# huangnengCSU/NanoSNP

Hardware: AMD Instinct MI355X
Metric: candidate SNP sites/sec (pileup encode + model fwd), 30x windows (higher is better)
Workload: dtype f32; 1 GPU; BASELINE configs[1]: pileup encode + PileupModel fwd, 1M synthetic 30x windows (G2) resident in HBM, batch=4096; batch=4096, windows_resident_per_gpu=1048576, streams=32, precision=fp32, parallelism=site-sharded x1, rooted gather of calls, world_size_observed=1, gather=torch

## Files before the change

nanosnp_amd/csrc/nsnp_api.hip:

```cpp
#include "nsnp_common.hpp"

#include <new>

extern "C" int nsnp_version(void) { return 100; }

extern "C" const char* nsnp_strerror(int code)
{
    switch (code) {
    case NSNP_OK: return "ok";
    case NSNP_EINVAL: return "invalid argument";
    case NSNP_ENOMEM: return "out of memory";
    case NSNP_EHIP: return "HIP runtime error";
    case NSNP_ENOWEIGHTS: return "weights not loaded";
    case NSNP_EARCH: return "device is not gfx950";
    case NSNP_ESHAPE: return "unsupported model dimensions";
    case NSNP_ENOTSUP: return "optional component unavailable (RCCL not found)";
    case NSNP_ECOMM: return "RCCL call failed";
    default: return "unknown error";
    }
}

static hipError_t g_create_err = hipSuccess;

extern "C" int nsnp_last_hip_error(const nsnp_ctx* ctx, const char** text)
{
    const hipError_t e = ctx ? ctx->last_err : g_create_err;
    if (text) *text = hipGetErrorString(e);
    return (int)e;
}

extern "C" int nsnp_ctx_create(int device, nsnp_ctx** out)
{
    if (!out) return NSNP_EINVAL;
    *out = nullptr;
    nsnp_ctx* ctx = new (std::nothrow) nsnp_ctx();
    if (!ctx) return NSNP_ENOMEM;
    memset((void*)ctx, 0, sizeof(*ctx));
    ctx->device = device;
    ctx->last_err = hipSuccess;
    ctx->chunk_sites = 32768;
    ctx->hap_chunk = 16384;
    ctx->precision = 0;
    ctx->hap_precision = 0;
    ctx->cat_precision = 0;
    ctx->cat_conv_lds = 1;
    ctx->cat_conv_pix2 = 1;
    ctx->hap_b3x = 1;
    ctx->tok_fused = 0;
    ctx->proj1_tiles = 4;
    ctx->fused_l1 = 1;
    ctx->l0_rs = 1;
    ctx->l1_rs = 1;
    ctx->l1_stagger = 0;
    ctx->head_rs = 1;
    ctx->rs_prio = 0;
    hipDeviceProp_t prop;
    hipError_t e = hipSetDevice(device);
    if (e == hipSuccess) e = hipGetDeviceProperties(&prop, device);
    if (e != hipSuccess) { g_create_err = e; delete ctx; return NSNP_EHIP; }
    if (strncmp(prop.gcnArchName, "gfx950", 6) != 0) { delete ctx; return NSNP_EARCH; }
    ctx->n_cu = prop.multiProcessorCount;
    *out = ctx;
    return NSNP_OK;
}

void nsnp_hap_free(nsnp_ctx* ctx);
int  nsnp_hap_reserve(nsnp_ctx* ctx);
void nsnp_cat_free(nsnp_ctx* ctx);
void nsnp_tok_free(nsnp_ctx* ctx);

constexpr size_t TIMER_MAX_PAIRS = 8192;

ScopedKernelTimer::ScopedKernelTimer(nsnp_ctx* c, int kernel, hipStream_t stream)
    : ctx(c), k(kernel), s(stream), stop_ev(nullptr), on(false)
{
    KernelTimer* t = c->timer;
    if (!t || !t->enabled || t->used[k] >= TIMER_MAX_PAIRS) return;
    if (t->used[k] == t->start[k].size()) {
        hipEvent_t a, b;
        if (hipEventCreate(&a) != hipSuccess) return;
        if (hipEventCreate(&b) != hipSuccess) { (void)hipEventDestroy(a); return; }
        t->start[k].push_back(a); t->stop[k].push_back(b);
    }
    const size_t i = t->used[k]++;
    (void)hipEventRecord(t->start[k][i], s);
    stop_ev = t->stop[k][i];
    on = true;
}
void ScopedKernelTimer::stop() { if (on) { (void)hipEventRecord(stop_ev, s); on = false; } }
ScopedKernelTimer::~ScopedKernelTimer() { stop(); }

extern "C" int nsnp_ctx_set_option(nsnp_ctx* ctx, const char* name, int64_t value)
{
    if (!ctx || !name) return NSNP_EINVAL;
    if (strcmp(name, "cat_precision") == 0) {
        if (value != 0 && value != 1 && value != 2) return NSNP_EINVAL;
        ctx->cat_precision = (int)value;
        return NSNP_OK;
    }
    if (strcmp(name, "tok_fused") == 0) {
        if (value != 0 && value != 1) return NSNP_EINVAL;
        ctx->tok_fused = (int)value;
        return NSNP_OK;
    }
    if (strcmp(name, "hap_b3x") == 0) {
        if (value != 0 && value != 1) return NSNP_EINVAL;
        ctx->hap_b3x = (int)value;
        return NSNP_OK;
    }
    if (strcmp(name, "cat_conv_pix2") == 0) {
        if (value != 0 && value != 1) return NSNP_EINVAL;
        ctx->cat_conv_pix2 = (int)value;
        return NSNP_OK;
    }
    if (strcmp(name, "cat_conv_lds") == 0) {
        if (value != 0 && value != 1) return NSNP_EINVAL;
        ctx->cat_conv_lds = (int)value;
        return NSNP_OK;
    }
    if (strcmp(name, "hap_precision") == 0) {
        if (value != 0 && value != 1 && value != 2) return NSNP_EINVAL;
        ctx->hap_precision = (int)value;
        return nsnp_hap_reserve(ctx);
    }
    if (strcmp(name, "hap_pass_sites") == 0) {
        if (value < 128 || value > 131072 || value % 128) return NSNP_EINVAL;
        const int64_t old = ctx->hap_chunk;
        ctx->hap_chunk = value;
        const int rc = nsnp_hap_reserve(ctx);
        if (rc) { ctx->hap_chunk = old; (void)nsnp_hap_reserve(ctx); }
        return rc;
    }
    if (strcmp(name, "pileup_precision") == 0) {
        if (value != 0 && value != 1 && value != 2) return NSNP_EINVAL;
        ctx->precision = (int)value;
        if (value == 2 && ctx->ws_h0 && ctx->ws_h0_floats < 192) return nsnp_ctx_reserve(ctx, ctx->chunk_sites);
        return NSNP_OK;
    }
    if (strcmp(name, "fused_l1") == 0) {
        if (value != 0 && value != 1) return NSNP_EINVAL;
        ctx->fused_l1 = (int)value;
        return NSNP_OK;
    }
    if (strcmp(name, "l0_register_stationary") == 0) {
        if (value != 0 && value != 1) return NSNP_EINVAL;
        ctx->l0_rs = (int)value;
        return NSNP_OK;
    }
    if (strcmp(name, "l1_register_stationary") == 0) {
        if (value != 0 && value != 1 && value != 2) return NSNP_EINVAL;
        ctx->l1_rs = (int)value;
        return NSNP_OK;
    }
    if (strcmp(name, "l0_input_weights_in_lds") == 0) {
        if (value != 0 && value != 1) return NSNP_EINVAL;
        ctx->l0_wx_lds = (int)value;
        return NSNP_OK;
    }
    if (strcmp(name, "static_priority") == 0) {
        if (value < 0 || value > 3) return NSNP_EINVAL;
        ctx->rs_prio = (int)value;
        return NSNP_OK;
    }
    if (strcmp(name, "head_split") == 0) {
        if (value != 0 && value != 1) return NSNP_EINVAL;
        ctx->head_rs = (int)value;
        return NSNP_OK;
    }
    if (strcmp(name, "l1_stagger") == 0) {
        if (value != 0 && value != 1) return NSNP_EINVAL;
        ctx->l1_stagger = (int)value;
        return NSNP_OK;
    }
    if (strcmp(name, "l1_site_groups") == 0) {
        if (value != 0 && value != 1 && value != 2 && value != 4) return NSNP_EINVAL;
        ctx->l1_rs_groups = (int)value;
        return NSNP_OK;
    }
    if (strcmp(name, "l0_site_groups") == 0) {
        if (value != 0 && value != 1 && value != 2 && value != 4) return NSNP_EINVAL;
        ctx->l0_rs_groups = (int)value;
        return NSNP_OK;
    }
    if (strcmp(name, "fused_waves") == 0) {
        if (value != 0 && value != 4 && value != 8 && value != 12) return NSNP_EINVAL;
        ctx->fused_waves = (int)value;
        return NSNP_OK;
    }
    if (strcmp(name, "proj1_tiles") == 0) {
        if (value < 1 || value > 64) return NSNP_EINVAL;
        ctx->proj1_tiles = (int)value;
        return NSNP_OK;
    }
    if (strcmp(name, "recurrence_waves") == 0) {
        if (value != 0 && value != 1 && value != 2 && value != 4 && value != 8) return NSNP_EINVAL;
        ctx->force_wpb = (int)value;
        return NSNP_OK;
    }
// ... 163 lines not shown
```

nanosnp_amd/csrc/nsnp_common.hpp:

```cpp
#pragma once

#include <hip/hip_runtime.h>
#include <stdint.h>
#include <stdlib.h>
#include <string.h>
#include <vector>

#include "nanosnp.h"

typedef float f32x4 __attribute__((ext_vector_type(4)));
typedef int   i32x4 __attribute__((ext_vector_type(4)));

#define NSNP_CDIV(a, b) (((a) + (b) - 1) / (b))

constexpr int PW = NSNP_PILEUP_WINDOW;
constexpr int PC = NSNP_PILEUP_CHANNELS;
constexpr int PH = 64;
constexpr int PG = 4 * PH;
constexpr int PCENTER = 16;
constexpr int PSTEPS1 = PCENTER + 1;


struct PileupWeightsDev {
    float* l0_whh[2];
    float* l0_wih[2];
    float* l0_wlast[2];
    float* l1_wih[2];
    float* l1_bias[2];
    float* l1_bias_raw[2];
    float* l1_whh[2];
    float* proj_w;
    float* proj_b;
    float* dense_w;
    float* dense_b;
    float* head_w;
    float* head_b;
    float* arena;
    size_t arena_bytes;
    bool   loaded;
};

struct PileupWeightsF16 {
    void* l0_whh[2]; void* l0_wih_hi[2]; void* l0_wih_lo[2]; void* l1_wih[2]; void* l1_whh[2];
    void* l1f_hi[2]; void* l1f_lo[2]; float* l1f_bias;
    void* l0_wih_rs[2];
    void* l1_wih_rs[2]; void* l1_whh_rs[2];
    void* l0_whh_rs[2];
    void* proj_w; void* dense_w; void* head_w;
    void* arena; size_t arena_bytes; bool loaded;
};

struct PileupWeightsB3 {
    void* l0_whh[2]; void* l0_wih[2]; void* l1_wih[2]; void* l1_whh[2];
    void* proj_w; void* dense_w; void* head_w;
    float* proj_b; float* dense_b; float* head_b;
    void* arena; size_t arena_bytes; bool loaded;
};

struct HapWeightsDev;
struct CatWeightsDev;

enum { NSNP_K_L0 = 0, NSNP_K_PROJ1, NSNP_K_L1, NSNP_K_HEAD, NSNP_K_ENCODE, NSNP_K_HAPFEAT, NSNP_K_HAPLSTM, NSNP_K_CATCONV, NSNP_K_CAT,
       NSNP_K_COUNT };
struct KernelTimer {
    std::vector<hipEvent_t> start[NSNP_K_COUNT], stop[NSNP_K_COUNT];
    size_t used[NSNP_K_COUNT];
    bool enabled;
};

struct PostOut { uint8_t* gt_arg; uint8_t* zy_arg; float* gt_max; float* zy_max; };

struct nsnp_ctx {
    int device;
    int n_cu;
    hipError_t last_err;
    bool attr_set;
    bool attr_set_f16;
    bool attr_set_b3;
    int hap_b3x;
// ... 68 lines not shown
```

nanosnp_amd/csrc/pileup_forward.hip:

```cpp
#include "nsnp_common.hpp"
#include "nsnp_lstm_cell.hpp"
#include "nsnp_devclock.hpp"

namespace {

constexpr float LOG2E = 1.4426950408889634f;

__device__ __forceinline__ f32x4 mfma4(float a, float b, f32x4 c)
{
    return __builtin_amdgcn_mfma_f32_16x16x4f32(a, b, c, 0, 0, 0);
}
__device__ __forceinline__ float sigmoid_f(float x)
{
    return __builtin_amdgcn_rcpf(1.0f + __builtin_amdgcn_exp2f(-LOG2E * x));
}
__device__ __forceinline__ float tanh_f(float x)
{
    return __builtin_fmaf(-2.0f, __builtin_amdgcn_rcpf(1.0f + __builtin_amdgcn_exp2f((2.0f * LOG2E) * x)), 1.0f);
}

__device__ __forceinline__ float lstm_cell(float zi, float zf, float zg, float zo, float& c)
{
    float cn;
    const float h = nsnp_cell::lstm_cell(zi, zf, zg, zo, c, cn);
    c = cn;
    return h;
}

template <int NT, int NJ4, int J4B, int J4N, int TB = 0, typename WP>
__device__ __forceinline__ void wave_gemm(WP w, int lane, const float* b, f32x4* acc)
{
#pragma unroll
    for (int j = 0; j < J4N; ++j) {
#pragma unroll
        for (int ig = 0; ig < NT; ig += 4) {
            f32x4 a[4];
#pragma unroll
            for (int u = 0; u < 4; ++u) a[u] = w[((TB + ig + u) * NJ4 + (J4B + j)) * 64 + lane];
#pragma unroll
            for (int e = 0; e < 4; ++e)
#pragma unroll
                for (int u = 0; u < 4; ++u) acc[ig + u] = mfma4(a[u][e], b[4 * j + e], acc[ig + u]);
            __builtin_amdgcn_sched_barrier(0);
        }
    }
}

__device__ __forceinline__ void wave_gemm2x16(const f32x4* w, int lane, const float* b, f32x4* acc)
{
#pragma unroll
    for (int j = 0; j < 16; ++j) {
        const f32x4 a0 = w[(0 * 16 + j) * 64 + lane], a1 = w[(1 * 16 + j) * 64 + lane];
#pragma unroll
        for (int e = 0; e < 4; ++e) {
            acc[0] = mfma4(a0[e], b[4 * j + e], acc[0]);
// ... 363 lines not shown
            const float* xr = &xx[cur][(16 * sg + n) * RS_XSROW];
            const f32x4 xb = *reinterpret_cast<const f32x4*>(xr + 4 * q);
            const float xl = xr[16 + q];
            f32x4 acc[4];
#pragma unroll
            for (int u = 0; u < 4; ++u) acc[u] = f32x4{0.f, 0.f, 0.f, 0.f};
            if (WXL) {
#pragma unroll
                for (int u = 0; u < 4; ++u) {
                    Wih[u] = *reinterpret_cast<const f32x4*>(&wxl[((wave * 4 + u) * 64 + lane) * 4]);
                    Wl[u] = wxl[4 * 4 * 64 * 4 + (wave * 4 + u) * 64 + lane];
                }
            }
#pragma unroll
            for (int e = 0; e < 4; ++e)
#pragma unroll
                for (int u = 0; u < 4; ++u) acc[u] = mfma4(Wih[u][e], xb[e], acc[u]);
#pragma unroll
            for (int u = 0; u < 4; ++u) acc[u] = mfma4(Wl[u], xl, acc[u]);
            if (s > 0) {
#define RS_KBLOCK(J, HB)                                                                               \
                _Pragma("unroll") for (int e = 0; e < 4; ++e)                                          \
                    _Pragma("unroll") for (int u = 0; u < 4; ++u) acc[u] = mfma4(Whh[u][J][e], HB[e], acc[u]);
                __builtin_amdgcn_sched_barrier(0);
                RS_KBLOCK(0, hb0)
                __builtin_amdgcn_sched_barrier(0);
                hb0 = *reinterpret_cast<const f32x4*>(hr + 32);
                RS_KBLOCK(1, hb1)
                __builtin_amdgcn_sched_barrier(0);
                hb1 = *reinterpret_cast<const f32x4*>(hr + 48);
                RS_KBLOCK(2, hb0)
                __builtin_amdgcn_sched_barrier(0);
                RS_KBLOCK(3, hb1)
#undef RS_KBLOCK
            }
            f32x4 hn;
#pragma unroll
            for (int u = 0; u < 4; ++u) {
                hn[u] = lstm_cell(acc[u][0], acc[u][1], acc[u][2], acc[u][3], c[sg][u]);
            }
            *reinterpret_cast<f32x4*>(&hx[cur][16 * sg + n][16 * wave + 4 * q]) = hn;
        }
        }
        if (s + 1 < PW) {
            stage_x(cur ^ 1);
            if (s + 2 < PW) load_x(dir ? t - 2 : t + 2);
        }
        lds_barrier();
    }
    flush_h((PW - 1) & 1, dir ? 0 : PW - 1);
    NSNP_DEVCLK_STOP(0)
}

constexpr int rs32_l1_lds_bytes(int nsg) { return (2 * 16 * nsg * RS_H0ROW + 2 * 16 * nsg * RS_XROW) * 4; }

template <int NSG, bool STAGGER>
__global__ __launch_bounds__(512, 2) void k_pileup_l1_rs32(
    const float* __restrict__ H0, int64_t N,
    const float* __restrict__ wih0, const float* __restrict__ wih1,
    const float* __restrict__ whh0, const float* __restrict__ whh1,
    const float* __restrict__ bias0, const float* __restrict__ bias1,
    float* __restrict__ H1c)
{
    extern __shared__ f32x4 lds[];
    constexpr int NS = 16 * NSG;
    float* const h0s = reinterpret_cast<float*>(lds);
    float* const h1x = h0s + 2 * NS * RS_H0ROW;
    const int dir = blockIdx.y;
    const int tid = threadIdx.x, lane = tid & 63, wave = tid >> 6;
    const int n = lane & 15, q = lane >> 4;
    const int64_t base_site = (int64_t)blockIdx.x * NS;

    f32x4 Wih[2][8], Whh[2][4], bias[2];
    {
        const f32x4* __restrict__ gih = reinterpret_cast<const f32x4*>(dir ? wih1 : wih0);
        const f32x4* __restrict__ ghh = reinterpret_cast<const f32x4*>(dir ? whh1 : whh0);
        const f32x4* __restrict__ gb = reinterpret_cast<const f32x4*>(dir ? bias1 : bias0);
#pragma unroll
        for (int u = 0; u < 2; ++u) {
#pragma unroll
            for (int j = 0; j < 8; ++j) Wih[u][j] = gih[((2 * wave + u) * 8 + j) * 64 + lane];
#pragma unroll
            for (int j = 0; j < 4; ++j) Whh[u][j] = ghh[((2 * wave + u) * 4 + j) * 64 + lane];
            bias[u] = gb[(2 * wave + u) * 64 + lane];
        }
    }

    const int cid = tid & 31;
    const int slot = (cid & 16) + 4 * (cid & 3) + ((cid >> 2) & 3);
    f32x4 sreg[NSG];
    auto load_h0 = [&](int t) {
#pragma unroll
        for (int k = 0; k < NSG; ++k) {
            const int64_t site = base_site + (tid >> 5) + 16 * k;
            const int64_t sc = site < N ? site : N - 1;
            sreg[k] = *reinterpret_cast<const f32x4*>(H0 + (sc * PW + t) * 128 + 4 * cid);
        }
    };
    auto store_h0 = [&](int buf) {
#pragma unroll
        for (int k = 0; k < NSG; ++k)
            *reinterpret_cast<f32x4*>(h0s + ((size_t)buf * NS + (tid >> 5) + 16 * k) * RS_H0ROW + 4 * slot) = sreg[k];
    };
    auto tpos = [&](int u) { return dir ? PW - 1 - u : u; };
    load_h0(tpos(0)); store_h0(0);
    load_h0(tpos(1)); store_h0(1);
// ... 446 lines not shown
        int d = 0;
        for (int k = 0; k < 8; ++k) { const int v = c[idx[k]]; if (v < 0) d -= v; }
        depth[n] = d;
    }
}

}

namespace {

inline int gate_row(int row)
{
    const int i = row >> 4, r = row & 15, qp = r >> 2, g = r & 3;
    return g * PH + 4 * i + qp;
}
struct MatRef { const float* w; int ld; const float* b0; const float* b1; };

float f_whh(const void* u, int row, int k) { const MatRef* m = (const MatRef*)u; return m->w[gate_row(row) * m->ld + k]; }
float f_wih0(const void* u, int row, int k) { const MatRef* m = (const MatRef*)u; return m->w[gate_row(row) * m->ld + k]; }
inline int h_store_col(int k) { const int j = k >> 2, q = k & 3; return (j >> 4) * 64 + 4 * (j & 15) + q; }
float f_wih1(const void* u, int row, int k) { const MatRef* m = (const MatRef*)u; return m->w[gate_row(row) * m->ld + h_store_col(k)]; }
float f_proj(const void* u, int row, int k) { const MatRef* m = (const MatRef*)u; return m->w[row * m->ld + h_store_col(k)]; }
inline int acc_col(int k) { const int j = k >> 2, q = k & 3; return 16 * (j >> 2) + 4 * q + (j & 3); }
float f_dense(const void* u, int row, int k) { const MatRef* m = (const MatRef*)u; return m->w[row * m->ld + acc_col(k)]; }
struct HeadRef { const float* gt; const float* zy; };
float f_head(const void* u, int row, int k)
{
    const HeadRef* m = (const HeadRef*)u;
    if (row < 21) return m->gt[row * 256 + acc_col(k)];
    if (row < 24) return m->zy[(row - 21) * 256 + acc_col(k)];
    return 0.f;
}

}

void nsnp_pack_image(float* img, int n_tiles, int n_j4, nsnp_wfun f, const void* user)
{
    for (int tile = 0; tile < n_tiles; ++tile)
        for (int j4 = 0; j4 < n_j4; ++j4)
            for (int lane = 0; lane < 64; ++lane)
                for (int e = 0; e < 4; ++e) {
                    const int row = 16 * tile + (lane & 15);
                    const int k = 4 * (4 * j4 + e) + (lane >> 4);
                    img[(((size_t)tile * n_j4 + j4) * 64 + lane) * 4 + e] = f(user, row, k);
                }
}

int nsnp_pileup_pack_weights(nsnp_ctx* ctx, const float* const* w)
{
    PileupWeightsDev& pw = ctx->pw;
    const size_t n_whh = 16 * 4 * 256, n_wih0 = 16 * 1 * 256, n_wlast = 16 * 64, n_wih1 = 16 * 8 * 256,
                 n_b1 = 16 * 256, n_proj = 8 * 8 * 256, n_pb = 8 * 256, n_dense = 16 * 8 * 256, n_db = 16 * 256,
                 n_head = 2 * 16 * 256, n_hb = 2 * 256;
    const size_t total = 2 * (n_whh + n_wih0 + n_wlast + n_wih1 + 2 * n_b1 + n_whh) + n_proj + n_pb + n_dense + n_db + n_head + n_hb;
    std::vector<float> host(total);
    size_t off = 0;
    auto take = [&](size_t n) { float* p = host.data() + off; off += n; return p; };
    float* h_l0_whh[2]; float* h_l0_wih[2]; float* h_l0_wlast[2]; float* h_l1_wih[2]; float* h_l1_b[2]; float* h_l1_braw[2]; float* h_l1_whh[2];
    for (int d = 0; d < 2; ++d) {
        h_l0_whh[d] = take(n_whh); h_l0_wih[d] = take(n_wih0); h_l0_wlast[d] = take(n_wlast);
        h_l1_wih[d] = take(n_wih1); h_l1_b[d] = take(n_b1); h_l1_braw[d] = take(n_b1); h_l1_whh[d] = take(n_whh);
    }
    float* h_proj = take(n_proj); float* h_pb = take(n_pb); float* h_dense = take(n_dense); float* h_db = take(n_db);
    float* h_head = take(n_head); float* h_hb = take(n_hb);

    std::vector<float> scaled[16];
    const float* ws[16];
    for (int t = 0; t < 16; ++t) {
        const int layer = t / 8, kind = t % 4;
        const size_t cols = kind == 0 ? (layer ? 2 * PH : PC) : (kind == 1 ? PH : 1);
        scaled[t].resize((size_t)4 * PH * cols);
        for (int r = 0; r < 4 * PH; ++r) {
            const float f = (r / PH == 2) ? -2.0f * LOG2E : -LOG2E;
            for (size_t k = 0; k < cols; ++k) scaled[t][r * cols + k] = f * w[t][r * cols + k];
        }
        ws[t] = scaled[t].data();
    }
    for (int d = 0; d < 2; ++d) {
        const float* const* l0 = ws + d * 4;
        const float* const* l1 = ws + 8 + d * 4;
        MatRef m;
        m = MatRef{l0[1], PH, nullptr, nullptr};  nsnp_pack_image(h_l0_whh[d], 16, 4, f_whh, &m);
        m = MatRef{l0[0], PC, nullptr, nullptr};  nsnp_pack_image(h_l0_wih[d], 16, 1, f_wih0, &m);
        for (int tile = 0; tile < 16; ++tile)
            for (int lane = 0; lane < 64; ++lane) {
                const int tr = gate_row(16 * tile + (lane & 15)), kq = lane >> 4;
                float v = 0.f;
                if (kq < 2) v = l0[0][tr * PC + 16 + kq];
                else if (kq == 2) v = l0[2][tr] + l0[3][tr];
                h_l0_wlast[d][tile * 64 + lane] = v;
            }
        m = MatRef{l1[0], 2 * PH, nullptr, nullptr};  nsnp_pack_image(h_l1_wih[d], 16, 8, f_wih1, &m);
        for (int tile = 0; tile < 16; ++tile)
            for (int lane = 0; lane < 64; ++lane)
                for (int g = 0; g < 4; ++g) {
                    const int tr = gate_row(16 * tile + 4 * (lane >> 4) + g);
                    h_l1_b[d][(tile * 64 + lane) * 4 + g] = l1[2][tr] + l1[3][tr];
                    h_l1_braw[d][(tile * 64 + lane) * 4 + g] = w[8 + d * 4 + 2][tr] + w[8 + d * 4 + 3][tr];
                }
        m = MatRef{l1[1], PH, nullptr, nullptr};  nsnp_pack_image(h_l1_whh[d], 16, 4, f_whh, &m);
    }
    {
        MatRef m{w[16], 128, nullptr, nullptr};  nsnp_pack_image(h_proj, 8, 8, f_proj, &m);
        for (int tile = 0; tile < 8; ++tile) for (int lane = 0; lane < 64; ++lane) for (int g = 0; g < 4; ++g)
            h_pb[(tile * 64 + lane) * 4 + g] = w[17][16 * tile + 4 * (lane >> 4) + g];
        MatRef md{w[18], 128, nullptr, nullptr}; nsnp_pack_image(h_dense, 16, 8, f_dense, &md);
        for (int tile = 0; tile < 16; ++tile) for (int lane = 0; lane < 64; ++lane) for (int g = 0; g < 4; ++g)
            h_db[(tile * 64 + lane) * 4 + g] = w[19][16 * tile + 4 * (lane >> 4) + g];
        HeadRef hr{w[20], w[22]};  nsnp_pack_image(h_head, 2, 16, f_head, &hr);
        for (int tile = 0; tile < 2; ++tile) for (int lane = 0; lane < 64; ++lane) for (int g = 0; g < 4; ++g) {
            const int row = 16 * tile + 4 * (lane >> 4) + g;
            h_hb[(tile * 64 + lane) * 4 + g] = row < 21 ? w[21][row] : (row < 24 ? w[23][row - 21] : 0.f);
        }
    }
    if (pw.arena && pw.arena_bytes != total * sizeof(float)) { (void)hipFree(pw.arena); pw.arena = nullptr; }
    if (!pw.arena) {
        NSNP_HIP(ctx, hipMalloc((void**)&pw.arena, total * sizeof(float)));
        pw.arena_bytes = total * sizeof(float);
    }
    NSNP_HIP(ctx, hipMemcpy(pw.arena, host.data(), total * sizeof(float), hipMemcpyHostToDevice));
    auto dev = [&](const float* hp) { return pw.arena + (hp - host.data()); };
    for (int d = 0; d < 2; ++d) {
        pw.l0_whh[d] = dev(h_l0_whh[d]); pw.l0_wih[d] = dev(h_l0_wih[d]); pw.l0_wlast[d] = dev(h_l0_wlast[d]);
        pw.l1_wih[d] = dev(h_l1_wih[d]); pw.l1_bias[d] = dev(h_l1_b[d]); pw.l1_bias_raw[d] = dev(h_l1_braw[d]); pw.l1_whh[d] = dev(h_l1_whh[d]);
    }
    pw.proj_w = dev(h_proj); pw.proj_b = dev(h_pb); pw.dense_w = dev(h_dense); pw.dense_b = dev(h_db);
    pw.head_w = dev(h_head); pw.head_b = dev(h_hb);
    pw.loaded = true;
    return NSNP_OK;
}

static int set_lds_attr_once(nsnp_ctx* ctx)
{
    if (ctx->attr_set) return NSNP_OK;
    NSNP_HIP(ctx, hipFuncSetAttribute((const void*)k_pileup_l0<8>, hipFuncAttributeMaxDynamicSharedMemorySize, L0_LDS_BYTES));
    NSNP_HIP(ctx, hipFuncSetAttribute((const void*)k_pileup_l0<4>, hipFuncAttributeMaxDynamicSharedMemorySize, L0_LDS_BYTES));
    NSNP_HIP(ctx, hipFuncSetAttribute((const void*)k_pileup_l0<2>, hipFuncAttributeMaxDynamicSharedMemorySize, L0_LDS_BYTES));
    NSNP_HIP(ctx, hipFuncSetAttribute((const void*)k_pileup_l0<1>, hipFuncAttributeMaxDynamicSharedMemorySize, L0_LDS_BYTES));
    NSNP_HIP(ctx, hipFuncSetAttribute((const void*)k_pileup_proj1, hipFuncAttributeMaxDynamicSharedMemorySize, P1_LDS_BYTES));
    NSNP_HIP(ctx, hipFuncSetAttribute((const void*)k_pileup_l1<8>, hipFuncAttributeMaxDynamicSharedMemorySize, L1_LDS_BYTES));
    NSNP_HIP(ctx, hipFuncSetAttribute((const void*)k_pileup_l1<4>, hipFuncAttributeMaxDynamicSharedMemorySize, L1_LDS_BYTES));
    NSNP_HIP(ctx, hipFuncSetAttribute((const void*)k_pileup_l1<2>, hipFuncAttributeMaxDynamicSharedMemorySize, L1_LDS_BYTES));
    NSNP_HIP(ctx, hipFuncSetAttribute((const void*)k_pileup_l1<1>, hipFuncAttributeMaxDynamicSharedMemorySize, L1_LDS_BYTES));
    NSNP_HIP(ctx, hipFuncSetAttribute((const void*)k_pileup_l1_rs4<1>, hipFuncAttributeMaxDynamicSharedMemorySize, rs4_l1_lds_bytes(1)));
    NSNP_HIP(ctx, hipFuncSetAttribute((const void*)k_pileup_l1_rs4<2>, hipFuncAttributeMaxDynamicSharedMemorySize, rs4_l1_lds_bytes(2)));
    NSNP_HIP(ctx, hipFuncSetAttribute((const void*)k_pileup_l1_rs32<4, true>, hipFuncAttributeMaxDynamicSharedMemorySize, rs32_l1_lds_bytes(4)));
    NSNP_HIP(ctx, hipFuncSetAttribute((const void*)k_pileup_l1_rs32<2, true>, hipFuncAttributeMaxDynamicSharedMemorySize, rs32_l1_lds_bytes(2)));
    NSNP_HIP(ctx, hipFuncSetAttribute((const void*)k_pileup_l1_rs32<4, false>, hipFuncAttributeMaxDynamicSharedMemorySize, rs32_l1_lds_bytes(4)));
    NSNP_HIP(ctx, hipFuncSetAttribute((const void*)k_pileup_l1_rs32<2, false>, hipFuncAttributeMaxDynamicSharedMemorySize, rs32_l1_lds_bytes(2)));
    ctx->attr_set = true;
    return NSNP_OK;
}

int nsnp_pileup_forward_impl(nsnp_ctx* ctx, const int32_t* x, const int64_t* center_idx,
                             int64_t N, float* gt, float* zy, const PostOut* post, bool* post_written, hipStream_t s)
{
    if (!ctx->pw.loaded) return NSNP_ENOWEIGHTS;
    if (N == 0) return NSNP_OK;
    int rc = set_lds_attr_once(ctx);
    if (rc) return rc;
    if (!ctx->ws_h0) { rc = nsnp_ctx_reserve(ctx, ctx->chunk_sites); if (rc) return rc; }
    const PileupWeightsDev& pw = ctx->pw;
    for (int64_t base = 0; base < N; base += ctx->chunk_sites) {
        const int64_t n = (N - base < ctx->chunk_sites) ? N - base : ctx->chunk_sites;
        const int32_t* xc = center_idx ? x : x + base * (PW * PC);
        const int64_t* cc = center_idx ? center_idx + base : nullptr;
        const int64_t waves_total = NSNP_CDIV(n, 16) * 2;
        int wpb = 8;
        while (wpb > 1 && waves_total / wpb < (int64_t)ctx->n_cu / 2) wpb >>= 1;
        if (ctx->force_wpb) wpb = ctx->force_wpb;
        const dim3 g_rec((unsigned)NSNP_CDIV(n, 16 * wpb), 2);
        if (ctx->l0_rs) {
            ScopedKernelTimer tm(ctx, NSNP_K_L0, s);
            int nsg = 1;
            if (ctx->l0_rs_groups) nsg = ctx->l0_rs_groups;
#define LAUNCH_RS(G) hipLaunchKernelGGL(k_pileup_l0_rs32<G>, dim3((unsigned)NSNP_CDIV(n, 16 * G), 2), dim3(256), 0, s, xc, cc, n, \
                           pw.l0_whh[0], pw.l0_whh[1], pw.l0_wih[0], pw.l0_wih[1], pw.l0_wlast[0], pw.l0_wlast[1], ctx->ws_h0)
            if (ctx->l0_wx_lds && nsg == 1)
                hipLaunchKernelGGL((k_pileup_l0_rs32<1, true>), dim3((unsigned)NSNP_CDIV(n, 16), 2), dim3(256), 0, s, xc, cc, n,
                                   pw.l0_whh[0], pw.l0_whh[1], pw.l0_wih[0], pw.l0_wih[1], pw.l0_wlast[0], pw.l0_wlast[1], ctx->ws_h0);
            else
            if (nsg == 4) LAUNCH_RS(4); else if (nsg == 2) LAUNCH_RS(2); else LAUNCH_RS(1);
#undef LAUNCH_RS
        } else
        { ScopedKernelTimer tm(ctx, NSNP_K_L0, s);
#define LAUNCH_L0(W) hipLaunchKernelGGL(k_pileup_l0<W>, g_rec, dim3(64 * W), L0_LDS_BYTES, s, xc, cc, n, \
                           pw.l0_whh[0], pw.l0_whh[1], pw.l0_wih[0], pw.l0_wih[1], pw.l0_wlast[0], pw.l0_wlast[1], ctx->ws_h0)
        if (wpb == 8) LAUNCH_L0(8); else if (wpb == 4) LAUNCH_L0(4); else if (wpb == 2) LAUNCH_L0(2); else LAUNCH_L0(1);
#undef LAUNCH_L0
        }
        if (ctx->l1_rs == 1) {
            ScopedKernelTimer tm(ctx, NSNP_K_L1, s);
            int g1 = 1;
            if (ctx->l1_rs_groups == 1 || ctx->l1_rs_groups == 2) g1 = ctx->l1_rs_groups;
#define LAUNCH_R4(G) hipLaunchKernelGGL(k_pileup_l1_rs4<G>, dim3((unsigned)NSNP_CDIV(n, 16 * G), 2), dim3(256), rs4_l1_lds_bytes(G), s, \
                           ctx->ws_h0, n, pw.l1_wih[0], pw.l1_wih[1], pw.l1_whh[0], pw.l1_whh[1], pw.l1_bias[0], pw.l1_bias[1], ctx->ws_h1c)
            if (g1 == 2) LAUNCH_R4(2); else LAUNCH_R4(1);
#undef LAUNCH_R4
        } else if (ctx->l1_rs == 2) {
            ScopedKernelTimer tm(ctx, NSNP_K_L1, s);
            int g1 = NSNP_CDIV(n, 64) * 2 >= (int64_t)ctx->n_cu ? 4 : 2;
            if (ctx->l1_rs_groups) g1 = ctx->l1_rs_groups;
#define LAUNCH_R1(G) hipLaunchKernelGGL((k_pileup_l1_rs32<G, ST>), dim3((unsigned)NSNP_CDIV(n, 16 * G), 2), dim3(512), rs32_l1_lds_bytes(G), s, \
                           ctx->ws_h0, n, pw.l1_wih[0], pw.l1_wih[1], pw.l1_whh[0], pw.l1_whh[1], pw.l1_bias[0], pw.l1_bias[1], ctx->ws_h1c)
            if (ctx->l1_stagger) { constexpr bool ST = true; if (g1 == 4) LAUNCH_R1(4); else LAUNCH_R1(2); }
            else { constexpr bool ST = false; if (g1 == 4) LAUNCH_R1(4); else LAUNCH_R1(2); }
#undef LAUNCH_R1
        } else {
        { const int rx = nsnp_ctx_need_xp1(ctx); if (rx) return rx; }
        const int64_t n_rt = NSNP_CDIV(n * PSTEPS1, 16);
        int64_t gp = NSNP_CDIV(n_rt, 16 * (int64_t)ctx->proj1_tiles);
        if (gp > ctx->n_cu) gp = ctx->n_cu;
        if (gp < 1) gp = 1;
        { ScopedKernelTimer tm(ctx, NSNP_K_PROJ1, s);
        hipLaunchKernelGGL(k_pileup_proj1, dim3((unsigned)gp, 2), dim3(1024), P1_LDS_BYTES, s, ctx->ws_h0, n,
                           pw.l1_wih[0], pw.l1_wih[1], pw.l1_bias[0], pw.l1_bias[1], ctx->ws_xp1); }
        { ScopedKernelTimer tm(ctx, NSNP_K_L1, s);
#define LAUNCH_L1(W) hipLaunchKernelGGL(k_pileup_l1<W>, g_rec, dim3(64 * W), L1_LDS_BYTES, s, ctx->ws_xp1, n, \
                           pw.l1_whh[0], pw.l1_whh[1], ctx->ws_h1c)
        if (wpb == 8) LAUNCH_L1(8); else if (wpb == 4) LAUNCH_L1(4); else if (wpb == 2) LAUNCH_L1(2); else LAUNCH_L1(1);
#undef LAUNCH_L1
        }
        }
        ScopedKernelTimer tm_head(ctx, NSNP_K_HEAD, s);
        if (ctx->head_rs) {
// ... 32 lines not shown
```

nanosnp_amd/csrc/pileup_forward_bf16x3.hip:

```cpp
#include "nsnp_common.hpp"
#include "nsnp_lstm_cell.hpp"
#include <type_traits>

namespace {

typedef __bf16 b8 __attribute__((ext_vector_type(8)));
typedef __bf16 b4 __attribute__((ext_vector_type(4)));
typedef __bf16 b2 __attribute__((ext_vector_type(2)));

__device__ __forceinline__ f32x4 mfma_b(b8 a, b8 b, f32x4 c)
{
    return __builtin_amdgcn_mfma_f32_16x16x32_bf16(a, b, c, 0, 0, 0);
}
__device__ __forceinline__ void split3(float v, __bf16& p0, __bf16& p1, __bf16& p2)
{
    p0 = (__bf16)v;
    const float r1 = v - (float)p0;
    p1 = (__bf16)r1;
    p2 = (__bf16)(r1 - (float)p1);
}
__device__ __forceinline__ void lds_barrier() { asm volatile("s_waitcnt lgkmcnt(0)\n\ts_barrier" ::: "memory"); }

template <int NT, int NB = 3>
__device__ __forceinline__ void six_products(const b8 (*a)[3], const b8* b, f32x4* acc)
{
    if (NB > 2) {
#pragma unroll
        for (int t = 0; t < NT; ++t) acc[t] = mfma_b(a[t][0], b[2], acc[t]);
    }
    if (NB > 1) {
#pragma unroll
        for (int t = 0; t < NT; ++t) acc[t] = mfma_b(a[t][1], b[1], acc[t]);
    }
#pragma unroll
    for (int t = 0; t < NT; ++t) acc[t] = mfma_b(a[t][2], b[0], acc[t]);
    if (NB > 1) {
#pragma unroll
        for (int t = 0; t < NT; ++t) acc[t] = mfma_b(a[t][0], b[1], acc[t]);
    }
#pragma unroll
    for (int t = 0; t < NT; ++t) acc[t] = mfma_b(a[t][1], b[0], acc[t]);
#pragma unroll
    for (int t = 0; t < NT; ++t) acc[t] = mfma_b(a[t][0], b[0], acc[t]);
}

constexpr int FR_H = 3 * 2 * 4 * 16 * 8;
constexpr int FR_X = 3 * 1 * 4 * 16 * 8;
constexpr int b3_l0_lds_bytes(int nsg) { return 2 * nsg * (FR_H + FR_X) * 2 + 64 + (nsg == 4 ? 4 * 4 * 64 * 16 : 0); }

template <int NSG>
__global__ __launch_bounds__(256, 2) void k_pileup_l0_b3(
    const int32_t* __restrict__ x, const int64_t* __restrict__ center_idx, int64_t N,
    const __bf16* __restrict__ whh0, const __bf16* __restrict__ whh1,
    const __bf16* __restrict__ wih0, const __bf16* __restrict__ wih1,
    __bf16* __restrict__ H0 )
{
    extern __shared__ b8 lds_b3[];
    __bf16* const hx = reinterpret_cast<__bf16*>(lds_b3);
    __bf16* const xx = hx + 2 * NSG * FR_H;
    int* const xflag = reinterpret_cast<int*>(xx + 2 * NSG * FR_X);
    constexpr bool CL = NSG == 4;
    f32x4* const cst = reinterpret_cast<f32x4*>(xflag + 16);
    const int dir = blockIdx.y;
    const int tid = threadIdx.x, lane = tid & 63, wave = tid >> 6;
    const int n = lane & 15, q = lane >> 4;

    b8 Whh[2][4][3], Wih[4][3];
    {
        const b8* __restrict__ ghh = reinterpret_cast<const b8*>(dir ? whh1 : whh0);
        const b8* __restrict__ gih = reinterpret_cast<const b8*>(dir ? wih1 : wih0);
#pragma unroll
        for (int u = 0; u < 4; ++u)
// ... 585 lines not shown
    sum += __shfl_xor(sum, 32);
    const float z1 = ah[1][1], z2 = ah[1][2], z3 = ah[1][3];
    const float zm = fmaxf(z1, fmaxf(z2, z3));
    const float ez1 = __expf(z1 - zm), ez2 = __expf(z2 - zm), ez3 = __expf(z3 - zm);
    const float zs = ez1 + ez2 + ez3;
    float p0[4], p1[4];
#pragma unroll
    for (int g = 0; g < 4; ++g) { p0[g] = e0[g] / sum; p1[g] = e1[g] / sum; }
    const float pz1 = ez1 / zs, pz2 = ez2 / zs, pz3 = ez3 / zs;
    if (live) {
        float* gp = gt_prob + site * NSNP_GT_CLASSES;
#pragma unroll
        for (int g = 0; g < 4; ++g) gp[4 * q + g] = p0[g];
        if (q == 0) {
#pragma unroll
            for (int g = 0; g < 4; ++g) gp[16 + g] = p1[g];
        }
        if (q == 1) {
            gp[20] = p1[0];
            float* zp = zy_prob + site * NSNP_ZY_CLASSES;
            zp[0] = pz1; zp[1] = pz2; zp[2] = pz3;
        }
    }
    if (gt_arg) {
        float bv = p0[0]; int bi = 4 * q;
#pragma unroll
        for (int g = 1; g < 4; ++g) if (p0[g] > bv) { bv = p0[g]; bi = 4 * q + g; }
        if (q == 0) {
#pragma unroll
            for (int g = 0; g < 4; ++g) if (p1[g] > bv) { bv = p1[g]; bi = 16 + g; }
        }
        if (q == 1 && p1[0] > bv) { bv = p1[0]; bi = 20; }
#pragma unroll
        for (int o = 16; o <= 32; o <<= 1) {
            const float ov = __shfl_xor(bv, o); const int oi = __shfl_xor(bi, o);
            if (ov > bv || (ov == bv && oi < bi)) { bv = ov; bi = oi; }
        }
        if (live && q == 0) { gt_arg[site] = (uint8_t)bi; gt_max[site] = bv; }
        if (live && q == 1) {
            float zb = pz1; int zi = 0;
            if (pz2 > zb) { zb = pz2; zi = 1; }
            if (pz3 > zb) { zb = pz3; zi = 2; }
            zy_arg[site] = (uint8_t)zi; zy_max[site] = zb;
        }
    }
}

}

namespace {

inline int gate_row(int row) { const int i = row >> 4, r = row & 15; return (r & 3) * PH + 4 * i + (r >> 2); }

inline uint16_t bf16_rne(float v)
{
    uint32_t u; memcpy(&u, &v, 4);
    if ((u & 0x7fffffffu) > 0x7f800000u) return (uint16_t)((u >> 16) | 0x40);
    return (uint16_t)((u + 0x7fffu + ((u >> 16) & 1u)) >> 16);
}
inline float bf16_f32(uint16_t h) { const uint32_t u = (uint32_t)h << 16; float v; memcpy(&v, &u, 4); return v; }

template <typename F>
void pack_b3(uint16_t* img, int n_tiles, int n_kb, F f)
{
    for (int tile = 0; tile < n_tiles; ++tile)
        for (int kb = 0; kb < n_kb; ++kb)
            for (int lane = 0; lane < 64; ++lane)
                for (int j = 0; j < 8; ++j) {
                    const float v = f(16 * tile + (lane & 15), kb, lane >> 4, j);
                    const uint16_t p0 = bf16_rne(v);
                    const float r1 = v - bf16_f32(p0);
                    const uint16_t p1 = bf16_rne(r1);
                    const uint16_t p2 = bf16_rne(r1 - bf16_f32(p1));
                    const size_t e = (((size_t)tile * n_kb + kb) * 3) * 64 + lane;
                    img[e * 8 + j] = p0;
                    img[(e + 64) * 8 + j] = p1;
                    img[(e + 128) * 8 + j] = p2;
                }
}

}

int nsnp_pileup_pack_weights_bf16(nsnp_ctx* ctx, const float* const* w)
{
    PileupWeightsB3& pw = ctx->pwb3;
    const size_t n_hh = (size_t)16 * 2 * 3 * 64 * 8, n_ih0 = (size_t)16 * 1 * 3 * 64 * 8, n_ih1 = (size_t)16 * 4 * 3 * 64 * 8;
    const size_t n_proj = (size_t)8 * 4 * 3 * 64 * 8, n_dense = (size_t)16 * 4 * 3 * 64 * 8, n_head = (size_t)2 * 8 * 3 * 64 * 8;
    const size_t total = 2 * (n_hh + n_ih0 + n_ih1 + n_hh) + n_proj + n_dense + n_head;
    std::vector<uint16_t> host(total);
    size_t off = 0;
    auto take = [&](size_t n) { uint16_t* p = host.data() + off; off += n; return p; };
    uint16_t *l0_hh[2], *l0_ih[2], *l1_ih[2], *l1_hh[2];
    for (int d = 0; d < 2; ++d) { l0_hh[d] = take(n_hh); l0_ih[d] = take(n_ih0); l1_ih[d] = take(n_ih1); l1_hh[d] = take(n_hh); }
    uint16_t* proj = take(n_proj); uint16_t* dense = take(n_dense); uint16_t* head = take(n_head);
    auto l0_unit = [](int p) { return 16 * (p >> 4) + 4 * (p & 3) + ((p >> 2) & 3); };
    auto l1_unit = [](int p) { return 4 * (2 * (p >> 3) + (p & 1)) + ((p >> 1) & 3); };
    auto acc_feat = [](int kb, int q, int j) { return 16 * (2 * kb + (j >> 2)) + 4 * q + (j & 3); };
    auto gs = [](int row) { return nsnp_cell::lstm_gate_scale(row); };
    for (int d = 0; d < 2; ++d) {
        const float* const* l0 = w + d * 4;
        const float* const* l1 = w + 8 + d * 4;
        pack_b3(l0_hh[d], 16, 2, [&](int row, int kb, int q, int j) { return gs(row) * l0[1][gate_row(row) * PH + l0_unit(32 * kb + 8 * q + j)]; });
        pack_b3(l0_ih[d], 16, 1, [&](int row, int, int q, int j) {
            const int tr = gate_row(row), k = 8 * q + j;
            if (k < PC) return gs(row) * l0[0][tr * PC + k];
            if (k == PC) return gs(row) * (l0[2][tr] + l0[3][tr]);
            return 0.f;
        });
        pack_b3(l1_ih[d], 16, 4, [&](int row, int kb, int q, int j) {
            return gs(row) * l1[0][gate_row(row) * 2 * PH + (kb >> 1) * PH + l0_unit(32 * (kb & 1) + 8 * q + j)]; });
        pack_b3(l1_hh[d], 16, 2, [&](int row, int kb, int q, int j) { return gs(row) * l1[1][gate_row(row) * PH + l1_unit(32 * kb + 8 * q + j)]; });
    }
    pack_b3(proj, 8, 4, [&](int row, int kb, int q, int j) { return w[16][row * 128 + 32 * kb + 8 * q + j]; });
    pack_b3(dense, 16, 4, [&](int row, int kb, int q, int j) { return w[18][row * 128 + acc_feat(kb, q, j)]; });
    pack_b3(head, 2, 8, [&](int row, int kb, int q, int j) {
        const int f = acc_feat(kb, q, j);
        if (row < 21) return w[20][row * 256 + f];
        if (row < 24) return w[22][(row - 21) * 256 + f];
        return 0.f;
    });
    float hb[128 + 256 + 32];
    for (int r = 0; r < 128; ++r) hb[r] = w[17][r];
    for (int r = 0; r < 256; ++r) hb[128 + r] = w[19][r];
    for (int r = 0; r < 32; ++r) hb[384 + r] = r < 21 ? w[21][r] : (r < 24 ? w[23][r - 21] : 0.f);
    const size_t wbytes = total * sizeof(uint16_t), bytes = wbytes + sizeof hb;
    if (pw.arena && pw.arena_bytes != bytes) { (void)hipFree(pw.arena); pw.arena = nullptr; }
    if (!pw.arena) { NSNP_HIP(ctx, hipMalloc((void**)&pw.arena, bytes)); pw.arena_bytes = bytes; }
    NSNP_HIP(ctx, hipMemcpy(pw.arena, host.data(), wbytes, hipMemcpyHostToDevice));
    NSNP_HIP(ctx, hipMemcpy((char*)pw.arena + wbytes, hb, sizeof hb, hipMemcpyHostToDevice));
    auto dev = [&](const uint16_t* hp) { return (void*)((char*)pw.arena + (hp - host.data()) * sizeof(uint16_t)); };
    for (int d = 0; d < 2; ++d) { pw.l0_whh[d] = dev(l0_hh[d]); pw.l0_wih[d] = dev(l0_ih[d]); pw.l1_wih[d] = dev(l1_ih[d]); pw.l1_whh[d] = dev(l1_hh[d]); }
    pw.proj_w = dev(proj); pw.dense_w = dev(dense); pw.head_w = dev(head);
// ... 70 lines not shown
```

Measured before the change: 19.66 million sites/s.

## Add register-stationary L0 LSTM kernel with bf16x3 MFMA input projection

Adds a new layer-0 LSTM kernel, now the default, that keeps the recurrent weights in registers. It computes the input projection with bf16 MFMA over a three-way bf16 split of the weights. Integer pileup inputs are staged into LDS as bf16, with an adaptive split level chosen per wave so small integers need only one plane. The bias is folded in as an extra input column set to 1. This is meant to remove the separate fp32 input-projection work and extra weight traffic, but it adds register pressure under a 3-wave occupancy bound and carries some precision risk from the bf16 split.

Result: faster. 20.38 million sites/s, median of 6 (+3.7%).

```diff
diff --git a/nanosnp_amd/csrc/nsnp_api.hip b/nanosnp_amd/csrc/nsnp_api.hip
--- a/nanosnp_amd/csrc/nsnp_api.hip
+++ b/nanosnp_amd/csrc/nsnp_api.hip
@@ -49,7 +49,7 @@
     ctx->tok_fused = 0;
     ctx->proj1_tiles = 4;
     ctx->fused_l1 = 1;
-    ctx->l0_rs = 1;
+    ctx->l0_rs = 2;
     ctx->l1_rs = 1;
     ctx->l1_stagger = 0;
     ctx->head_rs = 1;
@@ -143,7 +143,7 @@
         return NSNP_OK;
     }
     if (strcmp(name, "l0_register_stationary") == 0) {
-        if (value != 0 && value != 1) return NSNP_EINVAL;
+        if (value != 0 && value != 1 && value != 2) return NSNP_EINVAL;
         ctx->l0_rs = (int)value;
         return NSNP_OK;
     }
diff --git a/nanosnp_amd/csrc/nsnp_bf16.hpp b/nanosnp_amd/csrc/nsnp_bf16.hpp
--- /dev/null
+++ b/nanosnp_amd/csrc/nsnp_bf16.hpp
@@ -0,0 +1,48 @@
+#pragma once
+
+#include <hip/hip_runtime.h>
+#include <stdint.h>
+#include <string.h>
+
+typedef __bf16 b8 __attribute__((ext_vector_type(8)));
+typedef __bf16 b4 __attribute__((ext_vector_type(4)));
+typedef __bf16 b2 __attribute__((ext_vector_type(2)));
+
+namespace {
+
+__device__ __forceinline__ void split3(float v, __bf16& p0, __bf16& p1, __bf16& p2)
+{
+    p0 = (__bf16)v;
+    const float r1 = v - (float)p0;
+    p1 = (__bf16)r1;
+    p2 = (__bf16)(r1 - (float)p1);
+}
+
+inline uint16_t bf16_rne(float v)
+{
+    uint32_t u; memcpy(&u, &v, 4);
+    if ((u & 0x7fffffffu) > 0x7f800000u) return (uint16_t)((u >> 16) | 0x40);
+    return (uint16_t)((u + 0x7fffu + ((u >> 16) & 1u)) >> 16);
+}
+inline float bf16_f32(uint16_t h) { const uint32_t u = (uint32_t)h << 16; float v; memcpy(&v, &u, 4); return v; }
+
+template <typename F>
+void pack_b3(uint16_t* img, int n_tiles, int n_kb, F f)
+{
+    for (int tile = 0; tile < n_tiles; ++tile)
+        for (int kb = 0; kb < n_kb; ++kb)
+            for (int lane = 0; lane < 64; ++lane)
+                for (int j = 0; j < 8; ++j) {
+                    const float v = f(16 * tile + (lane & 15), kb, lane >> 4, j);
+                    const uint16_t p0 = bf16_rne(v);
+                    const float r1 = v - bf16_f32(p0);
+                    const uint16_t p1 = bf16_rne(r1);
+                    const uint16_t p2 = bf16_rne(r1 - bf16_f32(p1));
+                    const size_t e = (((size_t)tile * n_kb + kb) * 3) * 64 + lane;
+                    img[e * 8 + j] = p0;
+                    img[(e + 64) * 8 + j] = p1;
+                    img[(e + 128) * 8 + j] = p2;
+                }
+}
+
+}
diff --git a/nanosnp_amd/csrc/nsnp_common.hpp b/nanosnp_amd/csrc/nsnp_common.hpp
--- a/nanosnp_amd/csrc/nsnp_common.hpp
+++ b/nanosnp_amd/csrc/nsnp_common.hpp
@@ -25,6 +25,7 @@
     float* l0_whh[2];
     float* l0_wih[2];
     float* l0_wlast[2];
+    void*  l0_wx[2];
     float* l1_wih[2];
     float* l1_bias[2];
     float* l1_bias_raw[2];
diff --git a/nanosnp_amd/csrc/pileup_forward.hip b/nanosnp_amd/csrc/pileup_forward.hip
--- a/nanosnp_amd/csrc/pileup_forward.hip
+++ b/nanosnp_amd/csrc/pileup_forward.hip
@@ -1,6 +1,8 @@
 #include "nsnp_common.hpp"
 #include "nsnp_lstm_cell.hpp"
 #include "nsnp_devclock.hpp"
+#include "nsnp_bf16.hpp"
+#include <type_traits>
 
 namespace {
 
@@ -470,6 +472,151 @@
     NSNP_DEVCLK_STOP(0)
 }
 
+constexpr int RX_PLANE = 4 * 16 * 8;
+
+__global__ __launch_bounds__(256, 3) void k_pileup_l0_rsx(
+    const int32_t* __restrict__ x, const int64_t* __restrict__ center_idx, int64_t N,
+    const float* __restrict__ whh0, const float* __restrict__ whh1,
+    const __bf16* __restrict__ wx0, const __bf16* __restrict__ wx1,
+    float* __restrict__ H0)
+{
+    __shared__ __attribute__((aligned(16))) float hx[2][16][RS_XROW];
+    __shared__ __attribute__((aligned(16))) __bf16 xx[2][3][RX_PLANE];
+    __shared__ int xlvl[2][4];
+    __shared__ int64_t xofs[9 * 16];
+    const int dir = blockIdx.y;
+    const int tid = threadIdx.x, lane = tid & 63, wave = __builtin_amdgcn_readfirstlane(tid >> 6);
+    const int n = lane & 15, q = lane >> 4;
+    NSNP_DEVCLK_START
+    const int64_t base_site = (int64_t)blockIdx.x * 16;
+
+    f32x4 Whh[4][4];
+    b8 Wx[4][3];
+    {
+        const f32x4* __restrict__ ghh = reinterpret_cast<const f32x4*>(dir ? whh1 : whh0);
+        const b8* __restrict__ gx = reinterpret_cast<const b8*>(dir ? wx1 : wx0);
+#pragma unroll
+        for (int u = 0; u < 4; ++u) {
+#pragma unroll
+            for (int j = 0; j < 4; ++j) Whh[u][j] = ghh[((4 * wave + u) * 4 + j) * 64 + lane];
+#pragma unroll
+            for (int p = 0; p < 3; ++p) Wx[u][p] = gx[((4 * wave + u) * 3 + p) * 64 + lane];
+        }
+    }
+
+    const bool xon = tid < 9 * 16;
+    const int xrow = xon ? tid / 9 : 0, piece = xon ? tid % 9 : 0;
+    if (xon) {
+        const int64_t site = base_site + xrow;
+        const int64_t sc = site < N ? site : N - 1;
+        xofs[tid] = (center_idx ? (center_idx[sc] - PCENTER) * PC : sc * (PW * PC)) + 2 * piece;
+    }
+    int2 xi = int2{0, 0};
+    auto load_x = [&](int t) { if (xon) xi = *reinterpret_cast<const int2*>(x + xofs[tid] + t * PC); };
+    auto stage_x = [&](int buf) {
+        if (!xon) return;
+        int id = tid;
+        asm volatile("" : "+v"(id));
+        const int xdst = (id % 9 >> 2) * 128 + id / 9 * 8 + 2 * (id % 9 & 3);
+        const float f0 = (float)xi.x, f1 = (float)xi.y;
+        b2 p0, p1 = b2{0, 0}, p2 = b2{0, 0};
+        int lvl = 0;
+        const bool big = (unsigned)xi.x + 256u > 512u || (unsigned)xi.y + 256u > 512u;
+        if (__builtin_expect(__ballot(big) == 0ull, 1)) {
+            p0 = b2{(__bf16)f0, (__bf16)f1};
+        } else {
+            __bf16 a0, a1, a2, c0, c1, c2;
+            split3(f0, a0, a1, a2); split3(f1, c0, c1, c2);
+            p0 = b2{a0, c0}; p1 = b2{a1, c1}; p2 = b2{a2, c2};
+            const bool nz1 = (float)a1 != 0.f || (float)c1 != 0.f, nz2 = (float)a2 != 0.f || (float)c2 != 0.f;
+            lvl = __ballot(nz2) != 0ull ? 2 : (__ballot(nz1) != 0ull ? 1 : 0);
+        }
+        *reinterpret_cast<b2*>(&xx[buf][0][xdst]) = p0;
+        *reinterpret_cast<b2*>(&xx[buf][1][xdst]) = p1;
+        *reinterpret_cast<b2*>(&xx[buf][2][xdst]) = p2;
+        if (lane == 0) xlvl[buf][wave] = lvl;
+    };
+    for (int i = tid; i < 2 * 3 * RX_PLANE / 8; i += 256) reinterpret_cast<b8*>(&xx[0][0][0])[i] = b8{0, 0, 0, 0, 0, 0, 0, 0};
+    if (tid < 8) xlvl[tid >> 2][tid & 3] = 0;
+    __syncthreads();
+    if (tid < 32) xx[tid >> 4][0][2 * 128 + (tid & 15) * 8 + 2] = (__bf16)1.0f;
+    load_x(dir ? PW - 1 : 0);
+    stage_x(0);
+    if (PW > 1) load_x(dir ? PW - 2 : 1);
+    __syncthreads();
+
+    float c[4];
+#pragma unroll
+    for (int u = 0; u < 4; ++u) c[u] = 0.f;
+
+    float* const h0wg = H0 + (base_site * PW * 2 + dir) * 64;
+    const int nrows = (int)min((int64_t)16, N - base_site);
+    auto flush_h = [&](int buf, int t) {
+        int id = tid;
+        asm volatile("" : "+v"(id));
+        const int frow = id >> 4, fcid = id & 15;
+        if (frow < nrows)
+            *reinterpret_cast<f32x4*>(h0wg + frow * PW * 128 + t * 128 + 4 * fcid) =
+                *reinterpret_cast<const f32x4*>(&hx[buf][frow][16 * (fcid & 3) + 4 * (fcid >> 2)]);
+    };
+
+    for (int s = 0; s < PW; ++s) {
+        const int t = dir ? PW - 1 - s : s;
+        const int cur = s & 1;
+        if (s > 0) flush_h(cur ^ 1, dir ? t + 1 : t - 1);
+        const __bf16* xr = &xx[cur][0][q * 128 + n * 8];
+        const b8 xb0 = *reinterpret_cast<const b8*>(xr);
+        const int lvl = __builtin_amdgcn_readfirstlane(max(max(xlvl[cur][0], xlvl[cur][1]), max(xlvl[cur][2], xlvl[cur][3])));
+        f32x4 hn;
+        auto step = [&](auto lvl_tag) __attribute__((always_inline)) {
+            constexpr int LVL = decltype(lvl_tag)::value;
+            const float* hr = &hx[cur ^ 1][n][4 * q];
+            f32x4 hb0, hb1;
+            if (s > 0) { hb0 = *reinterpret_cast<const f32x4*>(hr); hb1 = *reinterpret_cast<const f32x4*>(hr + 16); }
+            f32x4 acc[4];
+#pragma unroll
+            for (int u = 0; u < 4; ++u) acc[u] = f32x4{0.f, 0.f, 0.f, 0.f};
+#pragma unroll
+            for (int p = LVL; p >= 0; --p) {
+                const b8 b = p ? *reinterpret_cast<const b8*>(xr + p * RX_PLANE) : xb0;
+#pragma unroll
+                for (int wp = 2; wp >= 0; --wp)
+#pragma unroll
+                    for (int u = 0; u < 4; ++u) acc[u] = __builtin_amdgcn_mfma_f32_16x16x32_bf16(Wx[u][wp], b, acc[u], 0, 0, 0);
+            }
+            if (s > 0) {
+#define RS_KBLOCK(J, HB)                                                                               \
+                _Pragma("unroll") for (int e = 0; e < 4; ++e)                                          \
+                    _Pragma("unroll") for (int u = 0; u < 4; ++u) acc[u] = mfma4(Whh[u][J][e], HB[e], acc[u]);
+                __builtin_amdgcn_sched_barrier(0);
+                RS_KBLOCK(0, hb0)
+                __builtin_amdgcn_sched_barrier(0);
+                hb0 = *reinterpret_cast<const f32x4*>(hr + 32);
+                RS_KBLOCK(1, hb1)
+                __builtin_amdgcn_sched_barrier(0);
+                hb1 = *reinterpret_cast<const f32x4*>(hr + 48);
+                RS_KBLOCK(2, hb0)
+                __builtin_amdgcn_sched_barrier(0);
+                RS_KBLOCK(3, hb1)
+#undef RS_KBLOCK
+            }
+#pragma unroll
+            for (int u = 0; u < 4; ++u) hn[u] = lstm_cell(acc[u][0], acc[u][1], acc[u][2], acc[u][3], c[u]);
+        };
+        if (__builtin_expect(lvl == 0, 1)) step(std::integral_constant<int, 0>{});
+        else if (lvl == 1)                 step(std::integral_constant<int, 1>{});
+        else                               step(std::integral_constant<int, 2>{});
+        *reinterpret_cast<f32x4*>(&hx[cur][n][16 * wave + 4 * q]) = hn;
+        if (s + 1 < PW) {
+            stage_x(cur ^ 1);
+            if (s + 2 < PW) load_x(dir ? t - 2 : t + 2);
+        }
+        lds_barrier();
+    }
+    flush_h((PW - 1) & 1, dir ? 0 : PW - 1);
+    NSNP_DEVCLK_STOP(0)
+}
+
 constexpr int rs32_l1_lds_bytes(int nsg) { return (2 * 16 * nsg * RS_H0ROW + 2 * 16 * nsg * RS_XROW) * 4; }
 
 template <int NSG, bool STAGGER>
@@ -1022,13 +1169,15 @@
     const size_t n_whh = 16 * 4 * 256, n_wih0 = 16 * 1 * 256, n_wlast = 16 * 64, n_wih1 = 16 * 8 * 256,
                  n_b1 = 16 * 256, n_proj = 8 * 8 * 256, n_pb = 8 * 256, n_dense = 16 * 8 * 256, n_db = 16 * 256,
                  n_head = 2 * 16 * 256, n_hb = 2 * 256;
-    const size_t total = 2 * (n_whh + n_wih0 + n_wlast + n_wih1 + 2 * n_b1 + n_whh) + n_proj + n_pb + n_dense + n_db + n_head + n_hb;
+    const size_t n_wx = 16 * 3 * 64 * 8 / 2;
+    const size_t total = 2 * (n_whh + n_wih0 + n_wlast + n_wx + n_wih1 + 2 * n_b1 + n_whh) + n_proj + n_pb + n_dense + n_db + n_head + n_hb;
     std::vector<float> host(total);
     size_t off = 0;
     auto take = [&](size_t n) { float* p = host.data() + off; off += n; return p; };
-    float* h_l0_whh[2]; float* h_l0_wih[2]; float* h_l0_wlast[2]; float* h_l1_wih[2]; float* h_l1_b[2]; float* h_l1_braw[2]; float* h_l1_whh[2];
+    float* h_l0_whh[2]; float* h_l0_wih[2]; float* h_l0_wlast[2]; float* h_l0_wx[2];
+    float* h_l1_wih[2]; float* h_l1_b[2]; float* h_l1_braw[2]; float* h_l1_whh[2];
     for (int d = 0; d < 2; ++d) {
-        h_l0_whh[d] = take(n_whh); h_l0_wih[d] = take(n_wih0); h_l0_wlast[d] = take(n_wlast);
+        h_l0_whh[d] = take(n_whh); h_l0_wih[d] = take(n_wih0); h_l0_wlast[d] = take(n_wlast); h_l0_wx[d] = take(n_wx);
         h_l1_wih[d] = take(n_wih1); h_l1_b[d] = take(n_b1); h_l1_braw[d] = take(n_b1); h_l1_whh[d] = take(n_whh);
     }
     float* h_proj = take(n_proj); float* h_pb = take(n_pb); float* h_dense = take(n_dense); float* h_db = take(n_db);
@@ -1060,6 +1209,10 @@
                 else if (kq == 2) v = l0[2][tr] + l0[3][tr];
                 h_l0_wlast[d][tile * 64 + lane] = v;
             }
+        pack_b3(reinterpret_cast<uint16_t*>(h_l0_wx[d]), 16, 1, [&](int row, int, int q, int j) {
+            const int k = 8 * q + j, tr = gate_row(row);
+            return k < PC ? l0[0][tr * PC + k] : (k == PC ? l0[2][tr] + l0[3][tr] : 0.f);
+        });
         m = MatRef{l1[0], 2 * PH, nullptr, nullptr};  nsnp_pack_image(h_l1_wih[d], 16, 8, f_wih1, &m);
         for (int tile = 0; tile < 16; ++tile)
             for (int lane = 0; lane < 64; ++lane)
@@ -1092,6 +1245,7 @@
     auto dev = [&](const float* hp) { return pw.arena + (hp - host.data()); };
     for (int d = 0; d < 2; ++d) {
         pw.l0_whh[d] = dev(h_l0_whh[d]); pw.l0_wih[d] = dev(h_l0_wih[d]); pw.l0_wlast[d] = dev(h_l0_wlast[d]);
+        pw.l0_wx[d] = dev(h_l0_wx[d]);
         pw.l1_wih[d] = dev(h_l1_wih[d]); pw.l1_bias[d] = dev(h_l1_b[d]); pw.l1_bias_raw[d] = dev(h_l1_braw[d]); pw.l1_whh[d] = dev(h_l1_whh[d]);
     }
     pw.proj_w = dev(h_proj); pw.proj_b = dev(h_pb); pw.dense_w = dev(h_dense); pw.dense_b = dev(h_db);
@@ -1140,7 +1294,11 @@
         while (wpb > 1 && waves_total / wpb < (int64_t)ctx->n_cu / 2) wpb >>= 1;
         if (ctx->force_wpb) wpb = ctx->force_wpb;
         const dim3 g_rec((unsigned)NSNP_CDIV(n, 16 * wpb), 2);
-        if (ctx->l0_rs) {
+        if (ctx->l0_rs == 2) {
+            ScopedKernelTimer tm(ctx, NSNP_K_L0, s);
+            hipLaunchKernelGGL(k_pileup_l0_rsx, dim3((unsigned)NSNP_CDIV(n, 16), 2), dim3(256), 0, s, xc, cc, n,
+                               pw.l0_whh[0], pw.l0_whh[1], (const __bf16*)pw.l0_wx[0], (const __bf16*)pw.l0_wx[1], ctx->ws_h0);
+        } else if (ctx->l0_rs) {
             ScopedKernelTimer tm(ctx, NSNP_K_L0, s);
             int nsg = 1;
             if (ctx->l0_rs_groups) nsg = ctx->l0_rs_groups;
diff --git a/nanosnp_amd/csrc/pileup_forward_bf16x3.hip b/nanosnp_amd/csrc/pileup_forward_bf16x3.hip
--- a/nanosnp_amd/csrc/pileup_forward_bf16x3.hip
+++ b/nanosnp_amd/csrc/pileup_forward_bf16x3.hip
@@ -1,23 +1,13 @@
 #include "nsnp_common.hpp"
 #include "nsnp_lstm_cell.hpp"
+#include "nsnp_bf16.hpp"
 #include <type_traits>
 
 namespace {
 
-typedef __bf16 b8 __attribute__((ext_vector_type(8)));
-typedef __bf16 b4 __attribute__((ext_vector_type(4)));
-typedef __bf16 b2 __attribute__((ext_vector_type(2)));
-
 __device__ __forceinline__ f32x4 mfma_b(b8 a, b8 b, f32x4 c)
 {
     return __builtin_amdgcn_mfma_f32_16x16x32_bf16(a, b, c, 0, 0, 0);
-}
-__device__ __forceinline__ void split3(float v, __bf16& p0, __bf16& p1, __bf16& p2)
-{
-    p0 = (__bf16)v;
-    const float r1 = v - (float)p0;
-    p1 = (__bf16)r1;
-    p2 = (__bf16)(r1 - (float)p1);
 }
 __device__ __forceinline__ void lds_barrier() { asm volatile("s_waitcnt lgkmcnt(0)\n\ts_barrier" ::: "memory"); }
 
@@ -709,32 +699,6 @@
 
 inline int gate_row(int row) { const int i = row >> 4, r = row & 15; return (r & 3) * PH + 4 * i + (r >> 2); }
 
-inline uint16_t bf16_rne(float v)
-{
-    uint32_t u; memcpy(&u, &v, 4);
-    if ((u & 0x7fffffffu) > 0x7f800000u) return (uint16_t)((u >> 16) | 0x40);
-    return (uint16_t)((u + 0x7fffu + ((u >> 16) & 1u)) >> 16);
-}
-inline float bf16_f32(uint16_t h) { const uint32_t u = (uint32_t)h << 16; float v; memcpy(&v, &u, 4); return v; }
-
-template <typename F>
-void pack_b3(uint16_t* img, int n_tiles, int n_kb, F f)
-{
-    for (int tile = 0; tile < n_tiles; ++tile)
-        for (int kb = 0; kb < n_kb; ++kb)
-            for (int lane = 0; lane < 64; ++lane)
-                for (int j = 0; j < 8; ++j) {
-                    const float v = f(16 * tile + (lane & 15), kb, lane >> 4, j);
-                    const uint16_t p0 = bf16_rne(v);
-                    const float r1 = v - bf16_f32(p0);
-                    const uint16_t p1 = bf16_rne(r1);
-                    const uint16_t p2 = bf16_rne(r1 - bf16_f32(p1));
-                    const size_t e = (((size_t)tile * n_kb + kb) * 3) * 64 + lane;
-                    img[e * 8 + j] = p0;
-                    img[(e + 64) * 8 + j] = p1;
-                    img[(e + 128) * 8 + j] = p2;
-                }
-}
 
 }
 
```
